# google/dynibar

Hardware: NVIDIA H100
Metric: rays/sec (64+64 samples x 8 src views) (higher is better)
Workload: dtype bf16

## Files before the change

dynibar_b200/csrc/chains_wg.cu:

```cuda
#include "nets.cuh"
#include "wg_engine.cuh"

namespace dyn {

using namespace tc;
using namespace fe;
using namespace wg;

namespace {

constexpr float kLog2e = 1.4426950408889634f, kLn2 = 0.6931471805599453f;

template <int RING>
struct ChainBars {
  static constexpr int kTileFull = 2 * RING, kTileEmpty = 2 * RING + 1, kCount = 2 * RING + 2;
};

template <int kTile, int kExtra, int kConst, int RING = kWgRing>
struct ChainSmem {
  static constexpr int kTileOff = RING * kWgStage;
  static constexpr int kExtraOff = kTileOff + kTile;
  static constexpr int kConstOff = kExtraOff + kExtra;
  static constexpr int kBarOff = (kConstOff + kConst * 4 + 7) & ~7;
  static constexpr int kBytes = kBarOff + ChainBars<RING>::kCount * 8;
// ... 227 lines not shown
    }
  }
#pragma unroll
  for (int s = 0; s < 8; ++s) acc_to_afrag(acc, s, ay[s]);
  float sg[2] = {0.f, 0.f};
  if (DYNAMIC) {
    named_bar_sync(1 + wg, 128);
    layer_rs_ss<256, 11, 8>(acc, ay, pe_pts, rg);
    {
      uint32_t ah[17][4];
      elu_log2_all<128>(acc);
#pragma unroll
      for (int s = 0; s < 16; ++s) acc_to_afrag(acc, s, ah[s]);
      bias_afrag(ah[16], 0, q);
      layer_rs<128, 17>(acc, ah, rg);
    }
    uint32_t ag[8][4];
    elu_log2_all<64>(acc);
    to_afrag<8>(acc, ag);
    layer_rs_ss<128, 10, 8>(acc, ag, pe_dir, rg);
#pragma unroll
    for (int j = 0; j < 16; ++j) {
      const float2 w = *reinterpret_cast<const float2*>(cst + C_WOG2 + 8 * j + 2 * q);
#pragma unroll
      for (int h = 0; h < 2; ++h)
        sg[h] = fmaf(elu_log2(acc[4 * j + 2 * h + 1]), w.y, fmaf(elu_log2(acc[4 * j + 2 * h]), w.x, sg[h]));
    }
    layer_rs_ss<128, 10, 8>(acc, ag, pe_dir, rg);
    elu_log2_all<64>(acc);
    to_afrag<8>(acc, ag);
    layer_rs_ss<64, 10, 8>(acc, ag, pe_dir, rg);
    float pr[3][2] = {{0.f, 0.f}, {0.f, 0.f}, {0.f, 0.f}};
#pragma unroll
    for (int j = 0; j < 8; ++j) {
#pragma unroll
      for (int h = 0; h < 2; ++h) {
        const float h0 = elu_log2(acc[4 * j + 2 * h]), h1 = elu_log2(acc[4 * j + 2 * h + 1]);
#pragma unroll
        for (int cc = 0; cc < 3; ++cc) {
          const float2 w = *reinterpret_cast<const float2*>(cst + C_WRGB4 + 64 * cc + 8 * j + 2 * q);
          pr[cc][h] = fmaf(h1, w.y, fmaf(h0, w.x, pr[cc][h]));
        }
      }
    }
#pragma unroll
    for (int h = 0; h < 2; ++h) {
      const float sigma = cst[C_BOG2] + quad_sum(sg[h]);
      const float r0 = cst[C_BRGB4] + quad_sum(pr[0][h]);
      const float r1 = cst[C_BRGB4 + 1] + quad_sum(pr[1][h]);
      const float r2 = cst[C_BRGB4 + 2] + quad_sum(pr[2][h]);
      if (q == 0 && ok[h]) {
        const bool none = nv[h] < 1.f;
        reinterpret_cast<float4*>(a.raw)[rows[h]] =
            make_float4(none ? 0.f : sigmoid_fast(r0), none ? 0.f : sigmoid_fast(r1),
                        none ? 0.f : sigmoid_fast(r2), none ? -1e9f : sigma - a.shift);
      }
    }
  } else {
    bias_afrag(ay[8], 0, q);
    layer_rs<128, 9>(acc, ay, rg);
#pragma unroll
    for (int j = 0; j < 16; ++j) {
      const float2 w = *reinterpret_cast<const float2*>(cst + C_WOG2 + 8 * j + 2 * q);
#pragma unroll
      for (int h = 0; h < 2; ++h)
        sg[h] = fmaf(elu_log2(acc[4 * j + 2 * h + 1]), w.y, fmaf(elu_log2(acc[4 * j + 2 * h]), w.x, sg[h]));
    }
    layer_rs<128, 9>(acc, ay, rg);
#pragma unroll
    for (int h = 0; h < 2; ++h) {
      const float sigma = cst[C_BOG2] + quad_sum(sg[h]);
      if (ok[h]) {
#pragma unroll
        for (int j = 0; j < 16; ++j)
          *f32_pair(a.GW, rows[h], 8 * j + 2 * q) = make_float2(acc[4 * j + 2 * h], acc[4 * j + 2 * h + 1]);
        if (q == 0) a.sigma[rows[h]] = nv[h] < 1.f ? -1e9f : sigma;
      }
    }
  }
}

template <bool DYNAMIC>
__global__ void __launch_bounds__(kWgThreads, 1) point2_wg_kernel(const __grid_constant__ Point2Args a) {
  extern __shared__ __align__(1024) uint8_t smem[];
  __shared__ __align__(16) FusedChunk s_tab[kWgMaxChunks];
  const uint32_t bar0 = chain_init(smem, P2Smem::kBarOff, s_tab, a.chunks, a.nchunks);
  float* cst = reinterpret_cast<float*>(smem + P2Smem::kConstOff);
  point2_constants(a, cst, DYNAMIC);
  __syncthreads();
  const int tid = threadIdx.x, lane = tid & 31;
  const int n_iter = (int)((a.P + 127) / 128);
  const int wg = __shfl_sync(0xffffffffu, tid >> 7, 0);
  if (wg == 2) {
    chain_producers(s_tab, a.nchunks, a.wimg, a.O, (uint32_t)kP2Tile, n_iter, smem, bar0);
    return;
  }
  setmaxnreg_inc<kConsumerRegs>();
  const int q = lane & 3, ww = (tid & 127) >> 5;
  const int fr[2] = {16 * ww + (lane >> 2), 16 * ww + (lane >> 2) + 8};
  Ring rg{smem, bar0, 0u, false, 0};
  const uint32_t tile = smem_u32(smem + P2Smem::kTileOff) + 1024u * wg;
  uint8_t* pe_pts = smem + P2Smem::kExtraOff + wg * (kPePtsBytes + kPeDirBytes);
  uint8_t* pe_dir = pe_pts + kPePtsBytes;
  uint32_t k = 0;
  for (int it = blockIdx.x; it < n_iter; it += gridDim.x, ++k) {
    const long long row0 = (long long)it * 128 + 64 * wg;
    if (DYNAMIC) {
      named_bar_sync(1 + wg, 128);
      write_pe_tiles(a, row0, pe_pts, pe_dir);
    }
    long long rows[2];
    bool ok[2];
    float nv[2];
    float2 res[2][16];
#pragma unroll
    for (int h = 0; h < 2; ++h) {
      rows[h] = row0 + fr[h];
      ok[h] = rows[h] < a.P;
      nv[h] = ok[h] ? a.nvalid[rows[h]] : 0.f;
#pragma unroll
      for (int j = 0; j < 16; ++j) res[h][j] = ok[h] ? __ldg(f32_pair(a.g2, rows[h], 8 * j + 2 * q)) : make_float2(0.f, 0.f);
    }
    float acc[128];
    tile_wait(bar0, k);
    layer_ss<128, 8, 128>(acc, tile, rg);
    layer_finish<128>(acc, rg);
    tile_release(bar0);
#pragma unroll
    for (int h = 0; h < 2; ++h)
#pragma unroll
      for (int j = 0; j < 16; ++j) {
        acc[4 * j + 2 * h] += res[h][j].x;
        acc[4 * j + 2 * h + 1] += res[h][j].y;
      }
    point2_heads<DYNAMIC>(acc, a, cst, smem_u32(pe_pts), smem_u32(pe_dir), rows, ok, nv, wg, rg);
  }
}

constexpr int kFusedRing = 5;
constexpr int kKvBytes = 2 * 128 * 256;
using FusedSmem = ChainSmem<kP1Tile, kKvBytes, kP2Const, kFusedRing>;
constexpr float kAttnScale = 0.17677669529663687f;

template <int KEYS, class W>
__device__ __forceinline__ void store_keys(uint8_t* dst, const int* kr, const bool* ok, int q, W word) {
#pragma unroll
  for (int h = 0; h < 2; ++h)
#pragma unroll
    for (int j = 0; j < 16; ++j)
      *reinterpret_cast<uint32_t*>(dst + j * (KEYS * 16) + (kr[h] >> 3) * 128 + (kr[h] & 7) * 16 + 4 * q) =
          ok[h] ? word(j, h) : 0u;
}

template <int KEYS>
__device__ __forceinline__ void attend(const uint32_t (&qf)[8][4], uint32_t (&of)[8][4], uint32_t kt, uint32_t vt,
                                       const float* sc, const int* lo, int S) {
  constexpr int NL = KEYS / 2, KG = KEYS * 16;
  const int q = threadIdx.x & 3;
  const bool part = S < KEYS;
#pragma unroll
  for (int hd = 0; hd < 4; ++hd) {
    float lg[NL];
    fence_regs<NL>(lg);
    wgmma_fence();
#pragma unroll
    for (int ks = 0; ks < 2; ++ks)
      WgmmaRS<KEYS>::mma(lg, qf[2 * hd + ks], smem_desc(kt + (2 * hd + ks) * 2 * KG, KG, 128u), ks ? 1u : 0u);
    wgmma_commit();
    wgmma_wait<0>();
    fence_regs<NL>(lg);
    float mx[2] = {-INFINITY, -INFINITY};
#pragma unroll
    for (int i = 0; i < NL; ++i) {
      const int h = (i >> 1) & 1, key = 8 * (i >> 2) + 2 * q + (i & 1);
      if (!part || (unsigned)(key - lo[h]) < (unsigned)S) mx[h] = fmaxf(mx[h], lg[i]);
    }
    float sh[2], den[2] = {0.f, 0.f};
#pragma unroll
    for (int h = 0; h < 2; ++h) {
      mx[h] = fmaxf(mx[h], __shfl_xor_sync(0xffffffffu, mx[h], 1));
      mx[h] = fmaxf(mx[h], __shfl_xor_sync(0xffffffffu, mx[h], 2));
      sh[h] = mx[h] * sc[h];
    }
#pragma unroll
    for (int i = 0; i < NL; ++i) {
      const int h = (i >> 1) & 1, key = 8 * (i >> 2) + 2 * q + (i & 1);
      float e = ex2f(fmaf(lg[i], sc[h], -sh[h]));
      if (part && (unsigned)(key - lo[h]) >= (unsigned)S) e = 0.f;
      lg[i] = e;
      den[h] += e;
    }
    uint32_t pf[KEYS / 16][4];
#pragma unroll
    for (int s = 0; s < KEYS / 16; ++s) acc_to_afrag(lg, s, pf[s]);
    float o[16];
    fence_regs<16>(o);
    wgmma_fence();
#pragma unroll
    for (int s = 0; s < KEYS / 16; ++s)
      WgmmaRS<32, 1>::mma(o, pf[s], smem_desc(vt + 4 * hd * KG + s * 256, 128u, KG), s ? 1u : 0u);
    wgmma_commit();
    wgmma_wait<0>();
    fence_regs<16>(o);
#pragma unroll
    for (int h = 0; h < 2; ++h) {
      const float inv = 1.f / quad_sum(den[h]);
#pragma unroll
      for (int j = 0; j < 4; ++j) {
        o[4 * j + 2 * h] *= inv;
        o[4 * j + 2 * h + 1] *= inv;
      }
    }
    acc_to_afrag(o, 0, of[2 * hd]);
    acc_to_afrag(o, 1, of[2 * hd + 1]);
  }
}

__device__ __forceinline__ void afrag_to_image(const uint32_t (&af)[8][4], void* img, long long row0, const int* fr,
                                               int q, long long P) {
  uint8_t* o = reinterpret_cast<uint8_t*>(img);
#pragma unroll
  for (int h = 0; h < 2; ++h) {
    const long long row = row0 + fr[h];
    if (row >= P) continue;
#pragma unroll
    for (int s = 0; s < 8; ++s) {
      *reinterpret_cast<uint32_t*>(o + tile_image_off(row, 2 * s, 16) + 4 * q) = af[s][h];
      *reinterpret_cast<uint32_t*>(o + tile_image_off(row, 2 * s + 1, 16) + 4 * q) = af[s][2 + h];
    }
  }
}

template <bool DYNAMIC, int KEYS, bool CAPTURE>
__global__ void __launch_bounds__(kWgThreads, 1) point_fused_wg_kernel(const __grid_constant__ PointFusedArgs a) {
  extern __shared__ __align__(1024) uint8_t smem[];
  __shared__ __align__(16) FusedChunk s_tab[kWgMaxChunks];
  const Point1Args& p1 = a.p1;
  const Point2Args& p2 = a.p2;
  const uint32_t bar0 = chain_init<kFusedRing>(smem, FusedSmem::kBarOff, s_tab, p1.chunks, p1.nchunks);
  float* cst = reinterpret_cast<float*>(smem + FusedSmem::kConstOff);
  point2_constants(p2, cst, DYNAMIC);
  __syncthreads();
  const long long P = p1.P;
  const int S = p1.S;
  const int n_iter = (int)((P + 127) / 128);
  const int tid = threadIdx.x, lane = tid & 31;
  const int wg = __shfl_sync(0xffffffffu, tid >> 7, 0);
  if (wg == 2) {
    chain_producers<kFusedRing>(s_tab, p1.nchunks, p1.wimg, p1.G, (uint32_t)kP1Tile, n_iter, smem, bar0);
    return;
  }
  setmaxnreg_inc<kConsumerRegs>();
  const int q = lane & 3, ww = (tid & 127) >> 5;
  const int fr[2] = {16 * ww + (lane >> 2), 16 * ww + (lane >> 2) + 8};
  RingN<kFusedRing> rg{smem, bar0, 0u, false, 0};
  const uint32_t tile = smem_u32(smem + FusedSmem::kTileOff) + 1024u * wg;
  uint8_t* kt = smem + FusedSmem::kExtraOff + (KEYS == 64 ? wg * 32768 : 0);
  uint8_t* vt = kt + KEYS * 256;
  const int kr[2] = {(KEYS == 128 ? 64 * wg : 0) + fr[0], (KEYS == 128 ? 64 * wg : 0) + fr[1]};
  uint8_t* pe_pts = smem + FusedSmem::kExtraOff + wg * (KEYS == 64 ? 32768 : kPePtsBytes + kPeDirBytes);
  uint8_t* pe_dir = pe_pts + kPePtsBytes;
  auto kv_sync = [&]() {
    if (KEYS == 128) named_bar_sync(3, 256);
    else named_bar_sync(1 + wg, 128);
  };
  uint32_t k = 0;
  for (int it = blockIdx.x; it < n_iter; it += gridDim.x, ++k) {
    const long long row0 = (long long)it * 128 + 64 * wg;
    long long rows[2];
    bool ok[2];
    float nv[2];
#pragma unroll
    for (int h = 0; h < 2; ++h) {
      rows[h] = row0 + fr[h];
      ok[h] = rows[h] < P;
      nv[h] = ok[h] ? p2.nvalid[rows[h]] : 0.f;
    }
    float g2[64];
    uint32_t qf[8][4];
    {
      float acc[128];
      tile_wait<kFusedRing>(bar0, k);
      layer_ss<256, 17, 128>(acc, tile, rg);
      layer_finish<256>(acc, rg);
      tile_release<kFusedRing>(bar0);
      {
        uint32_t af[17][4];
        elu_log2_all<128>(acc);
#pragma unroll
        for (int s = 0; s < 16; ++s) acc_to_afrag(acc, s, af[s]);
        bias_afrag(af[16], 8, q);
        layer_rs<128, 17>(acc, af, rg);
      }
#pragma unroll
      for (int h = 0; h < 2; ++h) {
        const float* pe = p1.posenc ? p1.posenc + (ok[h] ? rows[h] % S : 0) * 128 : nullptr;
#pragma unroll
        for (int j = 0; j < 16; ++j) {
          const int c = 8 * j + 2 * q;
          float v0 = elu_from_log2(acc[4 * j + 2 * h]), v1 = elu_from_log2(acc[4 * j + 2 * h + 1]);
          if (pe) {
            const float2 p = __ldg(reinterpret_cast<const float2*>(pe + c));
            v0 += p.x;
            v1 += p.y;
          }
          g2[4 * j + 2 * h] = v0;
          g2[4 * j + 2 * h + 1] = v1;
          if (CAPTURE && ok[h]) *f32_pair(p1.g2, rows[h], c) = make_float2(v0, v1);
        }
      }
      uint32_t ag[8][4];
      to_afrag<8>(g2, ag);
      layer_rs<128, 8>(acc, ag, rg);
      to_afrag<8>(acc, qf);
      if (CAPTURE) store_image128(acc, p1.Q, row0, fr, q, P);
      kv_sync();
      auto pair = [&](int j, int h) { return pack_bf16x2(acc[4 * j + 2 * h], acc[4 * j + 2 * h + 1]); };
      layer_rs<128, 8>(acc, ag, rg);
      store_keys<KEYS>(kt, kr, ok, q, pair);
      if (CAPTURE) store_image128(acc, p1.K, row0, fr, q, P);
      layer_rs<128, 8>(acc, ag, rg);
      store_keys<KEYS>(vt, kr, ok, q, pair);
      if (CAPTURE) store_image128(acc, p1.V, row0, fr, q, P);
    }
    fence_proxy_async_smem();
    kv_sync();
    uint32_t of[8][4];
    {
      float sc[2];
      int lo[2];
#pragma unroll
      for (int h = 0; h < 2; ++h) {
        sc[h] = ok[h] && nv[h] > 1.f ? kAttnScale * kLog2e : 0.f;
        lo[h] = (kr[h] / S) * S;
      }
      attend<KEYS>(qf, of, smem_u32(kt), smem_u32(vt), sc, lo, S);
    }
    if (CAPTURE) afrag_to_image(of, a.O, row0, fr, q, P);
    if (DYNAMIC) {
      kv_sync();
      write_pe_tiles(p2, row0, pe_pts, pe_dir);
    }
    float acc[128];
    layer_rs<128, 8>(acc, of, rg);
#pragma unroll
    for (int i = 0; i < 64; ++i) acc[i] += g2[i];
    point2_heads<DYNAMIC>(acc, p2, cst, smem_u32(pe_pts), smem_u32(pe_dir), rows, ok, nv, wg, rg);
  }
}

template <int KEYS>
__global__ void __launch_bounds__(256, 1) attention_wg_kernel(const uint8_t* __restrict__ Q, const uint8_t* __restrict__ K,
                                                              const uint8_t* __restrict__ V,
                                                              const float* __restrict__ nvalid, long long P, int S,
                                                              uint8_t* __restrict__ O) {
  extern __shared__ __align__(1024) uint8_t smem[];
  const int tid = threadIdx.x, lane = tid & 31, wg = tid >> 7;
  const int q = lane & 3, ww = (tid & 127) >> 5;
  const int fr[2] = {16 * ww + (lane >> 2), 16 * ww + (lane >> 2) + 8};
  const long long row0 = (long long)blockIdx.x * 128 + 64 * wg;
  long long rows[2];
  bool ok[2];
#pragma unroll
  for (int h = 0; h < 2; ++h) {
    rows[h] = row0 + fr[h];
    ok[h] = rows[h] < P;
  }
  auto word = [&](const uint8_t* img, int h, int g) {
    return *reinterpret_cast<const uint32_t*>(img + tile_image_off(rows[h], g, 16) + 4 * q);
  };
  uint8_t* kt = smem + (KEYS == 64 ? wg * 32768 : 0);
  uint8_t* vt = kt + KEYS * 256;
  const int kr[2] = {(KEYS == 128 ? 64 * wg : 0) + fr[0], (KEYS == 128 ? 64 * wg : 0) + fr[1]};
  uint32_t qf[8][4], of[8][4];
#pragma unroll
  for (int s = 0; s < 8; ++s)
#pragma unroll
    for (int h = 0; h < 2; ++h) {
      qf[s][h] = word(Q, h, 2 * s);
      qf[s][2 + h] = word(Q, h, 2 * s + 1);
    }
  store_keys<KEYS>(kt, kr, ok, q, [&](int j, int h) { return word(K, h, j); });
  store_keys<KEYS>(vt, kr, ok, q, [&](int j, int h) { return word(V, h, j); });
  fence_proxy_async_smem();
  __syncthreads();
  float sc[2];
  int lo[2];
#pragma unroll
  for (int h = 0; h < 2; ++h) {
    sc[h] = ok[h] && nvalid[rows[h]] > 1.f ? kAttnScale * kLog2e : 0.f;
    lo[h] = (kr[h] / S) * S;
  }
  attend<KEYS>(qf, of, smem_u32(kt), smem_u32(vt), sc, lo, S);
  afrag_to_image(of, O, row0, fr, q, P);
}

constexpr int kRhTile = 16 * 2048;
constexpr int kRhChunks = 5;
constexpr int kRhDepth = 3;
template <int VP>
__host__ __device__ constexpr int rh_gw_stride() { return (128 / VP) * 16 + 16; }
constexpr int kRhGw = 32 * rh_gw_stride<8>();
constexpr int C_RW4 = 0, C_RB4 = 64;
constexpr int kRhConst = 68;
struct RhSmem {
  static constexpr int kXOff = kRhChunks * kWgStage;
  static constexpr int kGwOff = kXOff + kRhDepth * kRhTile;
  static constexpr int kConstOff = kGwOff + kRhDepth * kRhGw;
  static constexpr int kBarOff = (kConstOff + kRhConst * 4 + 7) & ~7;
  static constexpr int kBytes = kBarOff + (1 + 2 * kRhDepth) * 8;
  static_assert(kBytes <= 227 * 1024, "shared memory of one CTA");
};
__device__ __forceinline__ uint32_t rh_full(uint32_t bar0, uint32_t slot) { return bar0 + 8u * (1 + slot); }
__device__ __forceinline__ uint32_t rh_empty(uint32_t bar0, uint32_t slot) {
  return bar0 + 8u * (1 + kRhDepth + slot);
}

template <int VP>
__device__ __forceinline__ void head_rows(const RgbHeadArgs& a, long long row0, const int* fr, long long* pl,
                                          bool* pt_ok, bool* valid, long long* m) {
#pragma unroll
  for (int h = 0; h < 2; ++h) {
    const int v = fr[h] & (VP - 1);
    pl[h] = (row0 + fr[h]) / VP;
    pt_ok[h] = pl[h] < a.P;
    valid[h] = pt_ok[h] && v < a.V;
    m[h] = pl[h] * a.V + v;
  }
}

struct HeadIn {
  float vis[2];
  float4 rd[2];
  float mk[2], c3[2][3], sig[2];
};
template <int VP>
__device__ __forceinline__ void head_load(const RgbHeadArgs& a, long long row0, const int* fr, int q, HeadIn& in) {
  long long pl[2], m[2];
  bool pt_ok[2], valid[2];
  head_rows<VP>(a, row0, fr, pl, pt_ok, valid, m);
#pragma unroll
  for (int h = 0; h < 2; ++h) {
    in.vis[h] = 0.f;
    in.rd[h] = make_float4(0.f, 0.f, 0.f, 0.f);
    if (valid[h] && q < 3) {
      in.vis[h] = a.vis2[m[h]];
      in.rd[h] = __ldg(reinterpret_cast<const float4*>(a.ray_diff) + m[h]);
    }
    in.mk[h] = 0.f;
    in.c3[h][0] = in.c3[h][1] = in.c3[h][2] = 0.f;
    if (valid[h]) {
      in.mk[h] = a.mask_eff[m[h]];
      in.c3[h][0] = a.rgb_in[m[h] * 3]; in.c3[h][1] = a.rgb_in[m[h] * 3 + 1]; in.c3[h][2] = a.rgb_in[m[h] * 3 + 2];
    }
    in.sig[h] = pt_ok[h] ? a.sigma[pl[h]] : 0.f;
  }
}

template <int VP>
__global__ void __launch_bounds__(kWgThreads, 1) rgbhead_wg_kernel(const __grid_constant__ RgbHeadArgs a) {
  extern __shared__ __align__(1024) uint8_t smem[];
  const uint32_t bar0 = smem_u32(smem + RhSmem::kBarOff);
  float* cst = reinterpret_cast<float*>(smem + RhSmem::kConstOff);
  const int tid = threadIdx.x, lane = tid & 31;
  if (tid == 0) {
    mbar_init(bar0, 1);
    for (int s = 0; s < kRhDepth; ++s) {
      mbar_init(rh_full(bar0, s), 1);
      mbar_init(rh_empty(bar0, s), 8);
    }
    mbar_fence_init();
  }
  for (int i = tid; i < 64; i += blockDim.x) cst[C_RW4 + i] = a.params[a.o_wrgb4 + i] * kLn2;
  if (tid == 0) cst[C_RB4] = a.params[a.o_brgb4];
  __syncthreads();
  const int n_iter = (int)((a.P * VP + 127) / 128);
  const int wg = __shfl_sync(0xffffffffu, tid >> 7, 0);
  if (wg == 2) {
    setmaxnreg_dec<kProducerRegs>();
    if ((tid & 127) == 0) {
      const uint8_t* w = reinterpret_cast<const uint8_t*>(a.wimg);
      uint32_t bytes = 0;
      for (int c = 0; c < kRhChunks; ++c) bytes += a.chunks[c].bytes;
      mbar_arrive_expect_tx(bar0, bytes);
      for (int c = 0; c < kRhChunks; ++c)
        bulk_g2s(smem_u32(smem + c * kWgStage), w + a.chunks[c].off, a.chunks[c].bytes, bar0);
      const uint8_t* x = reinterpret_cast<const uint8_t*>(a.X);
      const uint8_t* gw = reinterpret_cast<const uint8_t*>(a.GW);
      constexpr uint32_t kGwRow = (128 / VP) * 16;
// ... 317 lines not shown
```

dynibar_b200/csrc/view_wg.cu:

```cuda
#include "geometry.cuh"
#include "nets.cuh"
#include "wg_engine.cuh"

namespace dyn {

using namespace tc;
using namespace fe;
using namespace wg;

namespace {

constexpr int kPeBytes = 14 * 1024, kPoolBytes = 30 * 1024, kWgATile = kPeBytes + kPoolBytes;
constexpr int C_B1 = 0, C_B2 = 256, C_B3 = 304, C_B4 = 560, C_B5 = 688, C_B6 = 816, C_W6V = 944, C_B7 = 1072,
              C_W8 = 1200, C_MISC = 1328, C_DFEAT = 1332, C_CAMS = 1372, C_W1 = C_CAMS + 16 * kMaxViews,
              C_MK = C_W1 + 128, C_TGT = C_MK + 128, C_TBL = C_TGT + 3 * kMaxTargets;
constexpr int kWgConst = C_TBL + kMaxTargets * 16 / 4;
constexpr int kViewBars = 2 * kWgRing + 4;
constexpr int kWgSmem = kWgRing * kWgStage + 2 * kWgATile + kWgConst * 4 + 4  + kViewBars * 8;
static_assert(kWgSmem + kWgMaxChunks * 16 <= 227 * 1024, "shared memory of one CTA");
constexpr int kViewThreads = 4 * 128;
constexpr int kViewConsumerRegs = 208, kViewFrontRegs = 72, kViewProducerRegs = 24;

enum Phase {
  PH_FRONT, PH_BAR, PH_WEIGHTS, PH_F1, PH_F1_EPI, PH_F2, PH_F2_EPI, PH_F3, PH_F3_EPI, PH_F4, PH_F4_EPI, PH_F5,
  PH_F5_EPI, PH_F6, PH_F6_EPI, PH_F7, PH_F7_EPI, PH_POOL2, PH_HANDOFF,
  PH_T = 28, PH_W = 29, PH_ITERS = 30, PH_LIFE = 31
};
constexpr int kPhaseSlots = 32;
__shared__ long long s_phase[3][kPhaseSlots];
template <bool PROF>
struct PhaseClock {
  const ViewFusedArgs& a;
  int wg;
  __device__ __forceinline__ bool on() const {
    return PROF && a.dbg != nullptr && blockIdx.x == 0 && (threadIdx.x & 127) == 0;
  }
  __device__ __forceinline__ long long* c() const { return s_phase[wg]; }
  __device__ __forceinline__ void start() {
    if (!on()) return;
    for (int i = 0; i < kPhaseSlots; ++i) c()[i] = 0;
    c()[PH_T] = c()[PH_LIFE] = clock64();
  }
  __device__ __forceinline__ void mark(int ph, long long waits) {
    if (!on()) return;
    long long* s = c();
    const long long now = clock64();
    s[ph] += now - s[PH_T] - (waits - s[PH_W]);
    s[PH_WEIGHTS] += waits - s[PH_W];
    s[PH_T] = now;
    s[PH_W] = waits;
  }
  __device__ __forceinline__ void iteration() {
    if (on()) ++c()[PH_ITERS];
  }
  __device__ __forceinline__ void finish() {
    if (!on()) return;
    c()[PH_LIFE] = clock64() - c()[PH_LIFE];
    for (int i = 0; i < kPhaseSlots; ++i) a.dbg[kPhaseSlots * wg + i] = c()[i];
  }
};

__device__ __forceinline__ void pe_comp(float x, float* o) {
  float s, c;
  __sincosf(x, &s, &c);
  o[0] = x;
#pragma unroll
  for (int k = 0; k < 5; ++k) {
    o[1 + k] = c;
    o[6 + k] = s;
    const float s2 = 2.f * s * c, c2 = 1.f - 2.f * s * s;
    s = s2; c = c2;
  }
}

template <int KS>
__device__ __forceinline__ void layer_ss256(float* acc, uint32_t a_tile, Ring& rg) {
  layer_issue<256, KS>(acc, rg, [&](float* d, int ks, uint64_t bd, uint32_t sc) {
    const uint64_t ad = smem_desc(a_tile + ks * 2048u, 1024u, 128u);
    Wgmma<128, 0, 0>::mma(d, ad, bd, sc);
    Wgmma<128, 0, 0>::mma(d + 64, ad, bd + (2048u >> 4), sc);
  });
}

template <int N, int KS>
__device__ __forceinline__ void layer_rs_issue(float* acc, const uint32_t (&af)[KS][4], Ring& rg) {
  layer_issue<N, KS>(acc, rg, [&](float* d, int ks, uint64_t bd, uint32_t sc) { WgmmaRS<N>::mma(d, af[ks], bd, sc); });
}

__device__ __forceinline__ void named_bar_arrive(int id, int nthreads) {
  asm volatile("bar.arrive %0, %1;" ::"r"(id), "r"(nthreads) : "memory");
}

__device__ __forceinline__ void store2_64(uint8_t* tile, int r, int col, float x, float y) {
  *reinterpret_cast<uint32_t*>(tile + (col >> 3) * 1024 + (r >> 3) * 128 + (r & 7) * 16 + (col & 7) * 2) =
      pack_bf16x2(x, y);
}

template <int VP, bool ST, bool MC>
__device__ __forceinline__ void front_end(const ViewFusedArgs& a, const float* cst, int t, long long row0,
                                          uint8_t* pe_tile, uint8_t* pool_tile, float* s_w1, float* s_mk) {
  const int tw = t >> 6, r = t & 63, v = r & (VP - 1);
  uint8_t* arow_pe = pe_tile + (r >> 3) * 128 + (r & 7) * 16;
  uint8_t* arow_pool = pool_tile + (r >> 3) * 128 + (r & 7) * 16;
  const float wh = a.w_img, hh = a.h_img;
  const bool want_rgb = (tw == 0) || (ST && a.mask_rgb);

  const long long pl = (row0 + r) / VP;
  const bool pt_ok = pl < a.P;
  const bool valid = pt_ok && v < a.V;
  const long long m = pl * a.V + v;
  float p3[3] = {0.f, 0.f, 0.f};
  if (pt_ok) { p3[0] = a.pts[pl * 3]; p3[1] = a.pts[pl * 3 + 1]; p3[2] = a.pts[pl * 3 + 2]; }
  float q3[3] = {p3[0], p3[1], p3[2]};
  if (!ST && valid) {
    const float* qq = a.pts_seq + ((long long)v * a.seq_stride + pl) * 3;
    q3[0] = qq[0]; q3[1] = qq[1]; q3[2] = qq[2];
  }

  const int k = (MC && pt_ok && a.tgt_idx != nullptr) ? a.tgt_idx[(int)pl / a.S] : 0;
  const int vc = valid ? (MC ? reinterpret_cast<const uint8_t*>(cst + C_TBL)[16 * k + v] : v) : 0;
  const float* cam = cst + C_CAMS + 16 * vc;
  float pu, pv;
  bool front;
  project_point(cam, q3[0], q3[1], q3[2], pu, pv, front);
  const bool inb = (pu <= wh - 1.f) && (pu >= 0.f) && (pv <= hh - 1.f) && (pv >= 0.f);
  const float mask_proj = (valid && inb && front) ? 1.f : 0.f;

  float chv[24];
#pragma unroll
  for (int i = 0; i < 24; ++i) chv[i] = 0.f;
  float rgb[3] = {0.f, 0.f, 0.f};
  {
    const float gx = 2.f * pu / (wh - 1.f) - 1.f, gy = 2.f * pv / (hh - 1.f) - 1.f;
    const float fx = (gx + 1.f) * 0.5f * (float)(a.w - 1), fy = (gy + 1.f) * 0.5f * (float)(a.h - 1);
    const float x0f = floorf(fx), y0f = floorf(fy);
    const int x0 = (int)x0f, y0 = (int)y0f;
    const float ax = fx - x0f, ay = fy - y0f, bx = (x0f + 1.f) - fx, by = (y0f + 1.f) - fy;
    const uint16_t* base = a.feat_bf + (long long)vc * a.h * a.w * kC + 16 * tw;
#pragma unroll
    for (int dy = 0; dy < 2; ++dy) {
      uint4 tf[4];
      float tw4[2];
#pragma unroll
      for (int dx = 0; dx < 2; ++dx) {
        const int xi = x0 + dx, yi = y0 + dy;
        const bool in = valid && xi >= 0 && xi < a.w && yi >= 0 && yi < a.h;
        tw4[dx] = in ? (dx ? ax : bx) * (dy ? ay : by) : 0.f;
        const int xc = min(max(xi, 0), a.w - 1), yc = min(max(yi, 0), a.h - 1);
        const uint4* tp = reinterpret_cast<const uint4*>(base + ((long long)yc * a.w + xc) * kC);
        tf[2 * dx] = __ldg(tp);
        tf[2 * dx + 1] = __ldg(tp + 1);
      }
#pragma unroll
      for (int dx = 0; dx < 2; ++dx) {
#pragma unroll
        for (int hlf = 0; hlf < 2; ++hlf) {
          const uint4 qv = tf[2 * dx + hlf];
          const uint32_t u[4] = {qv.x, qv.y, qv.z, qv.w};
#pragma unroll
          for (int j = 0; j < 4; ++j) {
            const float lo = __uint_as_float(u[j] << 16), hi = __uint_as_float(u[j] & 0xffff0000u);
            if (tw == 0) {
              chv[3 + 8 * hlf + 2 * j] += lo * tw4[dx];
              chv[3 + 8 * hlf + 2 * j + 1] += hi * tw4[dx];
            } else {
              chv[8 * hlf + 2 * j] += lo * tw4[dx]; chv[8 * hlf + 2 * j + 1] += hi * tw4[dx];
            }
          }
        }
      }
    }
    if (want_rgb) {
      const float fx = (gx + 1.f) * 0.5f * (float)(a.W - 1), fy = (gy + 1.f) * 0.5f * (float)(a.H - 1);
      const float x0f = floorf(fx), y0f = floorf(fy);
      const int x0 = (int)x0f, y0 = (int)y0f;
      const float ax = fx - x0f, ay = fy - y0f, bx = (x0f + 1.f) - fx, by = (y0f + 1.f) - fy;
      const float* base = a.rgba + (long long)vc * a.H * a.W * 4;
      float4 tr[4];
      float twr[4];
#pragma unroll
      for (int dy = 0; dy < 2; ++dy)
#pragma unroll
        for (int dx = 0; dx < 2; ++dx) {
          const int xi = x0 + dx, yi = y0 + dy;
          const bool in = valid && xi >= 0 && xi < a.W && yi >= 0 && yi < a.H;
          twr[2 * dy + dx] = in ? (dx ? ax : bx) * (dy ? ay : by) : 0.f;
          const int xc = min(max(xi, 0), a.W - 1), yc = min(max(yi, 0), a.H - 1);
          tr[2 * dy + dx] = __ldg(reinterpret_cast<const float4*>(base + ((long long)yc * a.W + xc) * 4));
        }
#pragma unroll
      for (int tp = 0; tp < 4; ++tp) {
        rgb[0] += tr[tp].x * twr[tp]; rgb[1] += tr[tp].y * twr[tp]; rgb[2] += tr[tp].z * twr[tp];
      }
    }
  }

  float rd[4];
  {
    const float* tgt = a.cams.tgt;
    if (MC && ST) tgt = cst + C_TGT + 3 * k;
    float a0 = tgt[0] - p3[0], a1 = tgt[1] - p3[1], a2 = tgt[2] - p3[2];
    normalize3(a0, a1, a2);
    float b0 = cam[12] - q3[0], b1 = cam[13] - q3[1], b2 = cam[14] - q3[2];
    normalize3(b0, b1, b2);
    rd[0] = a0 - b0; rd[1] = a1 - b1; rd[2] = a2 - b2;
    rd[3] = a0 * b0 + a1 * b1 + a2 * b2;
    normalize3(rd[0], rd[1], rd[2]);
  }

  float mask = mask_proj;
  if (ST && a.mask_rgb) mask *= ((rgb[0] + rgb[1] + rgb[2]) > 1e-3f) ? 1.f : 0.f;
  if (tw == 0) {
    chv[0] = rgb[0]; chv[1] = rgb[1]; chv[2] = rgb[2];
    if (valid) {
      a.mask_proj[m] = mask_proj;
      if (ST) {
        a.mask_eff[m] = mask;
        reinterpret_cast<float4*>(a.ray_diff)[m] = make_float4(rd[0], rd[1], rd[2], rd[3]);
        a.rgb_in[m * 3] = rgb[0]; a.rgb_in[m * 3 + 1] = rgb[1]; a.rgb_in[m * 3 + 2] = rgb[2];
      }
    }
  }
  if (!ST) {
    const int c0 = tw == 0 ? 0 : 19, nc = tw == 0 ? 19 : 16;
#pragma unroll
    for (int i = 0; i < 19; ++i)
      if (i < nc) chv[i] = valid ? chv[i] + cst[C_DFEAT + c0 + i] : 0.f;
  }

  float w1;
  if (ST && a.anti_alias) {
    const float e = ex2f(cst[C_MISC + 2] * (rd[3] - 1.f) * 1.4426950408889634f);
    const float emin = group_min<VP>(valid ? e : INFINITY);
    w1 = valid ? (e - emin) * mask : 0.f;
  } else {
    w1 = mask;
  }
  w1 = w1 / (group_sum<VP>(w1) + 1e-8f);
  if (tw == 0) { s_w1[r] = w1; s_mk[r] = mask; }

#pragma unroll
  for (int g = 0; g < 3; ++g) {
    if (tw == 1 && g == 2) break;
    float o[24];
#pragma unroll
    for (int j = 0; j < 8; ++j) {
      const float fv = chv[8 * g + j];
      const float s1 = group_sum<VP>(w1 * fv);
      const float d = fv - s1;
      const float s2 = group_sum<VP>(w1 * d * d);
      o[j] = s1; o[8 + j] = s2; o[16 + j] = fv;
    }
    const int cb = 72 * tw + 24 * g;
    store8_64(arow_pool, cb, o);
    store8_64(arow_pool, cb + 8, o + 8);
    store8_64(arow_pool, cb + 16, o + 16);
  }
  if (!ST && tw == 1) {
    const float z[8] = {0.f, 0.f, 0.f, 0.f, 0.f, 0.f, 0.f, 0.f};
    store8_64(arow_pool, 120, z);
  }

  if (ST) {
    float pl6[6];
    {
      const float ox = cam[12], oy = cam[13], oz = cam[14];
      float dx = p3[0] - ox, dy = p3[1] - oy, dz = p3[2] - oz;
      normalize3(dx, dy, dz);
      pl6[0] = dx; pl6[1] = dy; pl6[2] = dz;
      pl6[3] = oy * dz - oz * dy;
      pl6[4] = oz * dx - ox * dz;
      pl6[5] = ox * dy - oy * dx;
    }
    float xin[56];
    if (tw == 0) {
      pe_comp(p3[0], xin);         store8_64(arow_pe, 0, xin);
      pe_comp(p3[1], xin + 11);    store8_64(arow_pe, 8, xin + 8);
      pe_comp(p3[2], xin + 22);    store8_64(arow_pe, 16, xin + 16); store8_64(arow_pe, 24, xin + 24);
      pe_comp(pl6[0], xin + 33);   store8_64(arow_pe, 32, xin + 32);
      pe_comp(pl6[1], xin + 44);   xin[55] = 0.f;
      store8_64(arow_pe, 40, xin + 40);  store8_64(arow_pe, 48, xin + 48);
    } else {
      pe_comp(pl6[2], xin);        store8_64(arow_pe, 56, xin);
      pe_comp(pl6[3], xin + 11);   store8_64(arow_pe, 64, xin + 8);
      pe_comp(pl6[4], xin + 22);   store8_64(arow_pe, 72, xin + 16); store8_64(arow_pe, 80, xin + 24);
      pe_comp(pl6[5], xin + 33);   store8_64(arow_pe, 88, xin + 32);
      xin[44] = rd[0]; xin[45] = rd[1]; xin[46] = rd[2]; xin[47] = rd[3];
#pragma unroll
      for (int i = 48; i < 56; ++i) xin[i] = 0.f;
      store8_64(arow_pe, 96, xin + 40);  store8_64(arow_pe, 104, xin + 48);
    }
  }
}

template <int VP, bool ST, bool MC, bool PROF>
__global__ void __launch_bounds__(kViewThreads, 1) view_wg_kernel(const __grid_constant__ ViewFusedArgs a) {
  extern __shared__ __align__(1024) uint8_t smem[];
  uint8_t* ring = smem;
  uint8_t* atiles = smem + kWgRing * kWgStage;
  float* cst = reinterpret_cast<float*>(atiles + 2 * kWgATile);
  uint64_t* bars = reinterpret_cast<uint64_t*>(smem + ((kWgRing * kWgStage + 2 * kWgATile + kWgConst * 4 + 7) & ~7));
  __shared__ __align__(16) FusedChunk s_tab[kWgMaxChunks];
  const int tid = threadIdx.x, lane = tid & 31;
  const int wg = __shfl_sync(0xffffffffu, tid >> 7, 0);
  const uint32_t bar0 = smem_u32(bars);
  const uint32_t tiles_full = bar0 + 8u * (2 * kWgRing), tiles_empty = tiles_full + 16u;
  stage_chunks(s_tab, a.chunks, a.nchunks);
  if (tid == 0) {
    for (int i = 0; i < kWgRing; ++i) {
      mbar_init(bar0 + 8u * i, 1);
      mbar_init(bar0 + 8u * (kWgRing + i), 8);
    }
    for (int c = 0; c < 2; ++c) {
      mbar_init(tiles_full + 8u * c, 128);
      mbar_init(tiles_empty + 8u * c, 4);
    }
    mbar_fence_init();
  }
  {
    const float* prm = a.params;
    for (int i = tid; i < 16 * kMaxViews; i += blockDim.x) {
      const int vv = i >> 4, j = i & 15;
      cst[C_CAMS + i] = j < 12 ? a.cams.P[vv][j] : (j < 15 ? a.cams.center[vv][j - 12] : 0.f);
    }
    for (int i = tid; i < 256; i += blockDim.x) {
      cst[C_B1 + i] = ST ? prm[a.o_b1 + i] : 0.f;
      cst[C_B3 + i] = prm[a.o_b3 + i];
    }
    for (int i = tid; i < 128; i += blockDim.x) {
      cst[C_B4 + i] = prm[a.o_b4 + i];
      cst[C_B5 + i] = prm[a.o_b5 + i];
      cst[C_B6 + i] = prm[a.o_b6 + i];
      cst[C_W6V + i] = prm[a.o_w6 + 128 * 128 + i];
      cst[C_B7 + i] = prm[a.o_b7 + i];
      cst[C_W8 + i] = prm[a.o_w8 + i];
    }
    if (tid < 48) cst[C_B2 + tid] = (ST && tid < kF) ? prm[a.o_b2 + tid] : 0.f;
    if (tid < 40) cst[C_DFEAT + tid] = (!ST && tid < kF) ? a.dfeat[tid] : 0.f;
    if (tid == 0) {
      cst[C_MISC + 0] = prm[a.o_b6 + 128];
      cst[C_MISC + 1] = prm[a.o_b8];
      cst[C_MISC + 2] = (ST && a.o_s >= 0) ? fabsf(prm[a.o_s]) : 0.f;
    }
    if (MC && ST && tid < 3 * kMaxTargets) cst[C_TGT + tid] = a.cams.tgts[tid / 3][tid % 3];
    if (MC && tid < kMaxTargets * 4)
      reinterpret_cast<uint32_t*>(cst + C_TBL)[tid] = reinterpret_cast<const uint32_t*>(&a.tbl[0][0])[tid];
  }
  __syncthreads();

  const long long n_rows = a.P * VP;
  const int n_iter = (int)((n_rows + 127) / 128);
  const int t = tid & 127;
  if (wg == 3) {
    setmaxnreg_dec<kViewProducerRegs>();
    if (t == 0) producer_loop<kWgRing, kWgStage>(s_tab, a.nchunks, a.wimg, n_iter, ring, bar0);
    return;
  }
  if (wg == 2) {
    setmaxnreg_dec<kViewFrontRegs>();
    PhaseClock<PROF || !ST> pc{a, 2};
    pc.start();
    uint32_t k = 0;
    for (int it = blockIdx.x; it < n_iter; it += gridDim.x, ++k) {
#pragma unroll 1
      for (int c = 0; c < 2; ++c) {
        if (k > 0) mbar_wait(tiles_empty + 8u * c, (k - 1) & 1);
        pc.mark(PH_HANDOFF, 0);
        front_end<VP, ST, MC>(a, cst, t, (long long)it * 128 + 64 * c, atiles + c * kWgATile,
                          atiles + c * kWgATile + kPeBytes, cst + C_W1 + 64 * c, cst + C_MK + 64 * c);
        fence_proxy_async_smem();
        mbar_arrive(tiles_full + 8u * c);
        pc.mark(PH_FRONT, 0);
      }
      pc.iteration();
    }
    pc.finish();
    return;
  }
  setmaxnreg_inc<kViewConsumerRegs>();

  const int ww = t >> 5, q = lane & 3;
  uint8_t* pool_tile = atiles + wg * kWgATile + kPeBytes;
  const uint32_t pe_addr = smem_u32(atiles + wg * kWgATile), pool_addr = smem_u32(pool_tile);
  const float* s_w1 = cst + C_W1 + 64 * wg;
  const float* s_mk = cst + C_MK + 64 * wg;
  const int fr[2] = {16 * ww + (lane >> 2), 16 * ww + (lane >> 2) + 8};

  PhaseClock<PROF || !ST> pc{a, wg};
  Ring rg{ring, bar0, 0u, pc.on(), 0};
  pc.start();
#define TS(ph) pc.mark(ph, rg.wait_cycles)
  auto in_turn = [&](auto issue, bool pass) {
    named_bar_sync(3 + wg, 256);
    TS(PH_BAR);
    issue();
    if (pass) named_bar_arrive(4 - wg, 256);
  };
  if (wg == 1) named_bar_arrive(3, 256);

  uint32_t k = 0;
  for (int it = blockIdx.x; it < n_iter; it += gridDim.x, ++k) {
    const long long row0 = (long long)it * 128 + 64 * wg;
    mbar_wait(tiles_full + 8u * wg, k & 1);
    TS(PH_HANDOFF);
    const float w1r[2] = {s_w1[fr[0]], s_w1[fr[1]]}, mk[2] = {s_mk[fr[0]], s_mk[fr[1]]};

    float acc[128];
    if (ST) {
      in_turn([&] { layer_ss256<7>(acc, pe_addr, rg); }, true);
      layer_finish<256>(acc, rg);
      TS(PH_F1);
      {
        uint32_t af[16][4];
        bias_elu<256>(acc, cst + C_B1, q);
        to_afrag<16>(acc, af);
        TS(PH_F1_EPI);
        in_turn([&] { layer_rs_issue<48, 16>(acc, af, rg); }, true);
        layer_finish<48>(acc, rg);
      }
      TS(PH_F2);
      float f[2][10];
#pragma unroll
      for (int h = 0; h < 2; ++h) {
        const long long prow = (row0 + fr[h]) / VP;
        const bool ok = prow < a.P && ((fr[h] & (VP - 1)) < a.V);
        const float* rf = a.ref_feat + (ok ? prow / a.S : 0) * kF;
#pragma unroll
        for (int j = 0; j < 5; ++j)
#pragma unroll
          for (int e = 0; e < 2; ++e) {
            const int n = 8 * j + 2 * q + e;
            f[h][2 * j + e] = (ok && n < kF) ? (acc[4 * j + 2 * h + e] + cst[C_B2 + n]) * __ldg(rf + n) : 0.f;
          }
      }
#pragma unroll
      for (int j = 0; j < 5; ++j) {
        float mu[2][2], va[2][2];
#pragma unroll
        for (int e = 0; e < 2; ++e) {
          const int i = 2 * j + e;
          float tv[2] = {w1r[0] * f[0][i], w1r[1] * f[1][i]}, s1[2], s2[2];
          views_sum<VP>(tv, s1);
          const float d0 = f[0][i] - s1[0], d1 = f[1][i] - s1[1];
          tv[0] = w1r[0] * d0 * d0;
          tv[1] = w1r[1] * d1 * d1;
          views_sum<VP>(tv, s2);
          mu[0][e] = s1[0]; mu[1][e] = s1[1]; va[0][e] = s2[0]; va[1][e] = s2[1];
        }
        const int n = 8 * j + 2 * q;
#pragma unroll
        for (int h = 0; h < 2; ++h) {
          store2_64(pool_tile, fr[h], 120 + n, mu[h][0], mu[h][1]);
          store2_64(pool_tile, fr[h], 160 + n, va[h][0], va[h][1]);
          store2_64(pool_tile, fr[h], 200 + n, f[h][2 * j], f[h][2 * j + 1]);
        }
      }
      TS(PH_F2_EPI);
      fence_proxy_async_smem();
      named_bar_sync(1 + wg, 128);
      TS(PH_BAR);
    }
    in_turn([&] { layer_ss256<ST ? 15 : 8>(acc, pool_addr, rg); }, true);
    layer_finish<256>(acc, rg);
    __syncwarp();
    if (lane == 0) mbar_arrive(tiles_empty + 8u * wg);
    TS(PH_F3);
    {
      uint32_t af[16][4];
      bias_elu<256>(acc, cst + C_B3, q);
      to_afrag<16>(acc, af);
      TS(PH_F3_EPI);
      in_turn([&] { layer_rs_issue<128, 16>(acc, af, rg); }, true);
      layer_finish<128>(acc, rg);
    }
    TS(PH_F4);
    float x[64];
    bias_elu<128>(acc, cst + C_B4, q);
#pragma unroll
    for (int i = 0; i < 64; ++i) x[i] = acc[i];
    {
      uint32_t af[8][4];
      to_afrag<8>(x, af);
      TS(PH_F4_EPI);
      in_turn([&] { layer_rs_issue<128, 8>(acc, af, rg); }, true);
      layer_finish<128>(acc, rg);
    }
    TS(PH_F5);
    float part[2] = {0.f, 0.f};
#pragma unroll
    for (int j = 0; j < 16; ++j) {
      const float2 b = *reinterpret_cast<const float2*>(cst + C_B5 + 8 * j + 2 * q);
      const float2 wv = *reinterpret_cast<const float2*>(cst + C_W6V + 8 * j + 2 * q);
#pragma unroll
      for (int h = 0; h < 2; ++h) {
        float& h0 = acc[4 * j + 2 * h];
        float& h1 = acc[4 * j + 2 * h + 1];
        h0 = elu_fast(fmaf(h0, w1r[h], b.x));
        h1 = elu_fast(fmaf(h1, w1r[h], b.y));
        part[h] = fmaf(h1, wv.y, fmaf(h0, wv.x, part[h]));
      }
    }
    part[0] = quad_sum(part[0]);
    part[1] = quad_sum(part[1]);
    {
      uint32_t af[8][4];
      to_afrag<8>(acc, af);
      TS(PH_F5_EPI);
      in_turn([&] { layer_rs_issue<128, 8>(acc, af, rg); }, true);
      layer_finish<128>(acc, rg);
    }
    TS(PH_F6);
    float vis1[2];
#pragma unroll
    for (int h = 0; h < 2; ++h) vis1[h] = sigmoid_fast(elu_fast(cst[C_MISC + 0] + part[h])) * mk[h];
    bias_elu<128>(acc, cst + C_B6, q);
#pragma unroll
    for (int i = 0; i < 64; ++i) x[i] += acc[i];
    {
      uint32_t af[8][4];
      to_afrag<8>(x, af);
      if (ST) {
        uint8_t* xo = reinterpret_cast<uint8_t*>(a.X);
#pragma unroll
        for (int s = 0; s < 8; ++s)
#pragma unroll
          for (int k = 0; k < 4; ++k)
            *reinterpret_cast<uint32_t*>(xo + tile_image_off(row0 + fr[k & 1], 2 * s + (k >> 1), 16) + 4 * q) = af[s][k];
      }
      TS(PH_F6_EPI);
      in_turn([&] { layer_rs_issue<128, 8>(acc, af, rg); }, wg == 0 || it + (int)gridDim.x < n_iter);
      layer_finish<128>(acc, rg);
    }
    TS(PH_F7);
    float p7[2] = {0.f, 0.f};
#pragma unroll
    for (int j = 0; j < 16; ++j) {
      const float2 b = *reinterpret_cast<const float2*>(cst + C_B7 + 8 * j + 2 * q);
      const float2 wv = *reinterpret_cast<const float2*>(cst + C_W8 + 8 * j + 2 * q);
#pragma unroll
      for (int h = 0; h < 2; ++h) {
        p7[h] = fmaf(elu_fast(fmaf(acc[4 * j + 2 * h], vis1[h], b.x)), wv.x, p7[h]);
        p7[h] = fmaf(elu_fast(fmaf(acc[4 * j + 2 * h + 1], vis1[h], b.y)), wv.y, p7[h]);
      }
    }
    float vis2[2];
#pragma unroll
// ... 178 lines not shown
```

Measured before the change: 257,300.

## Split dynamic attention into 64-key blocks and drop forced phase clock in non-ST path

In the dynamic fused chain, attention logits are now computed in 64-key blocks. The logits are recomputed in a second pass for the softmax-times-V product, which lowers the number of logit registers live at once. The cost is extra QK wgmma work. The view kernel also stops forcing the phase clock on in the non-ST variant and instead inserts a never-taken compiler barrier to keep instruction scheduling separated, cutting profiling overhead.

Measured after the change: 258,300, median of 6. About the same (+0.4%).

```diff
diff --git a/dynibar_b200/csrc/chains_wg.cu b/dynibar_b200/csrc/chains_wg.cu
--- a/dynibar_b200/csrc/chains_wg.cu
+++ b/dynibar_b200/csrc/chains_wg.cu
@@ -403,28 +403,36 @@
           ok[h] ? word(j, h) : 0u;
 }
 
-template <int KEYS>
+template <int KEYS, int KH = 64>
 __device__ __forceinline__ void attend(const uint32_t (&qf)[8][4], uint32_t (&of)[8][4], uint32_t kt, uint32_t vt,
                                        const float* sc, const int* lo, int S) {
-  constexpr int NL = KEYS / 2, KG = KEYS * 16;
+  static_assert(KH == 64 || KH == KEYS, "blocks of 64 keys or one block");
+  constexpr int NH = KEYS / KH, NL = KH / 2, KG = KEYS * 16;
   const int q = threadIdx.x & 3;
   const bool part = S < KEYS;
-#pragma unroll
-  for (int hd = 0; hd < 4; ++hd) {
-    float lg[NL];
+  auto logits = [&](float (&lg)[NL], int hd, int hf) {
     fence_regs<NL>(lg);
     wgmma_fence();
 #pragma unroll
     for (int ks = 0; ks < 2; ++ks)
-      WgmmaRS<KEYS>::mma(lg, qf[2 * hd + ks], smem_desc(kt + (2 * hd + ks) * 2 * KG, KG, 128u), ks ? 1u : 0u);
+      WgmmaRS<KH>::mma(lg, qf[2 * hd + ks], smem_desc(kt + (2 * hd + ks) * 2 * KG + hf * (KH * 16), KG, 128u),
+                       ks ? 1u : 0u);
     wgmma_commit();
     wgmma_wait<0>();
     fence_regs<NL>(lg);
+  };
+#pragma unroll
+  for (int hd = 0; hd < 4; ++hd) {
+    float lg[NL];
     float mx[2] = {-INFINITY, -INFINITY};
 #pragma unroll
-    for (int i = 0; i < NL; ++i) {
-      const int h = (i >> 1) & 1, key = 8 * (i >> 2) + 2 * q + (i & 1);
-      if (!part || (unsigned)(key - lo[h]) < (unsigned)S) mx[h] = fmaxf(mx[h], lg[i]);
+    for (int hf = 0; hf < NH; ++hf) {
+      logits(lg, hd, hf);
+#pragma unroll
+      for (int i = 0; i < NL; ++i) {
+        const int h = (i >> 1) & 1, key = KH * hf + 8 * (i >> 2) + 2 * q + (i & 1);
+        if (!part || (unsigned)(key - lo[h]) < (unsigned)S) mx[h] = fmaxf(mx[h], lg[i]);
+      }
     }
     float sh[2], den[2] = {0.f, 0.f};
 #pragma unroll
@@ -433,26 +441,31 @@
       mx[h] = fmaxf(mx[h], __shfl_xor_sync(0xffffffffu, mx[h], 2));
       sh[h] = mx[h] * sc[h];
     }
-#pragma unroll
-    for (int i = 0; i < NL; ++i) {
-      const int h = (i >> 1) & 1, key = 8 * (i >> 2) + 2 * q + (i & 1);
-      float e = ex2f(fmaf(lg[i], sc[h], -sh[h]));
-      if (part && (unsigned)(key - lo[h]) >= (unsigned)S) e = 0.f;
-      lg[i] = e;
-      den[h] += e;
-    }
-    uint32_t pf[KEYS / 16][4];
-#pragma unroll
-    for (int s = 0; s < KEYS / 16; ++s) acc_to_afrag(lg, s, pf[s]);
     float o[16];
-    fence_regs<16>(o);
-    wgmma_fence();
-#pragma unroll
-    for (int s = 0; s < KEYS / 16; ++s)
-      WgmmaRS<32, 1>::mma(o, pf[s], smem_desc(vt + 4 * hd * KG + s * 256, 128u, KG), s ? 1u : 0u);
-    wgmma_commit();
-    wgmma_wait<0>();
-    fence_regs<16>(o);
+#pragma unroll
+    for (int hf = 0; hf < NH; ++hf) {
+      if (NH > 1) logits(lg, hd, hf);
+#pragma unroll
+      for (int i = 0; i < NL; ++i) {
+        const int h = (i >> 1) & 1, key = KH * hf + 8 * (i >> 2) + 2 * q + (i & 1);
+        float e = ex2f(fmaf(lg[i], sc[h], -sh[h]));
+        if (part && (unsigned)(key - lo[h]) >= (unsigned)S) e = 0.f;
+        lg[i] = e;
+        den[h] += e;
+      }
+      uint32_t pf[KH / 16][4];
+#pragma unroll
+      for (int s = 0; s < KH / 16; ++s) acc_to_afrag(lg, s, pf[s]);
+      fence_regs<16>(o);
+      wgmma_fence();
+#pragma unroll
+      for (int s = 0; s < KH / 16; ++s)
+        WgmmaRS<32, 1>::mma(o, pf[s], smem_desc(vt + 4 * hd * KG + (KH / 16 * hf + s) * 256, 128u, KG),
+                            (hf | s) ? 1u : 0u);
+      wgmma_commit();
+      wgmma_wait<0>();
+      fence_regs<16>(o);
+    }
 #pragma unroll
     for (int h = 0; h < 2; ++h) {
       const float inv = 1.f / quad_sum(den[h]);
@@ -585,7 +598,7 @@
         sc[h] = ok[h] && nv[h] > 1.f ? kAttnScale * kLog2e : 0.f;
         lo[h] = (kr[h] / S) * S;
       }
-      attend<KEYS>(qf, of, smem_u32(kt), smem_u32(vt), sc, lo, S);
+      attend<KEYS, DYNAMIC ? 64 : KEYS>(qf, of, smem_u32(kt), smem_u32(vt), sc, lo, S);
     }
     if (CAPTURE) afrag_to_image(of, a.O, row0, fr, q, P);
     if (DYNAMIC) {
diff --git a/dynibar_b200/csrc/view_wg.cu b/dynibar_b200/csrc/view_wg.cu
--- a/dynibar_b200/csrc/view_wg.cu
+++ b/dynibar_b200/csrc/view_wg.cu
@@ -85,6 +85,10 @@
 template <int N, int KS>
 __device__ __forceinline__ void layer_rs_issue(float* acc, const uint32_t (&af)[KS][4], Ring& rg) {
   layer_issue<N, KS>(acc, rg, [&](float* d, int ks, uint64_t bd, uint32_t sc) { WgmmaRS<N>::mma(d, af[ks], bd, sc); });
+}
+
+__device__ __forceinline__ void block_split(bool never) {
+  if (never) asm volatile("" ::: "memory");
 }
 
 __device__ __forceinline__ void named_bar_arrive(int id, int nthreads) {
@@ -358,7 +362,7 @@
   }
   if (wg == 2) {
     setmaxnreg_dec<kViewFrontRegs>();
-    PhaseClock<PROF || !ST> pc{a, 2};
+    PhaseClock<PROF> pc{a, 2};
     pc.start();
     uint32_t k = 0;
     for (int it = blockIdx.x; it < n_iter; it += gridDim.x, ++k) {
@@ -386,12 +390,13 @@
   const float* s_mk = cst + C_MK + 64 * wg;
   const int fr[2] = {16 * ww + (lane >> 2), 16 * ww + (lane >> 2) + 8};
 
-  PhaseClock<PROF || !ST> pc{a, wg};
+  PhaseClock<PROF> pc{a, wg};
   Ring rg{ring, bar0, 0u, pc.on(), 0};
   pc.start();
 #define TS(ph) pc.mark(ph, rg.wait_cycles)
   auto in_turn = [&](auto issue, bool pass) {
     named_bar_sync(3 + wg, 256);
+    if (!ST) block_split(n_iter < 0);
     TS(PH_BAR);
     issue();
     if (pass) named_bar_arrive(4 - wg, 256);
```
